# Gadersd/stable-diffusion-burn

Measured on AMD Instinct MI355X. Metric: images/sec @512x512, 20-step DDIM CFG=7.5, SD v1.4, higher is better.
Workload: dtype f32

## Files before the change

### stable_diffusion_burn_amd/csrc/engine.cpp

```cpp
#include "engine.hpp"
#include "mpk_reader.hpp"

#include <dlfcn.h>

#include <algorithm>
#include <cmath>
#include <cstdarg>
#include <cstdio>
#include <cstring>
#include <fstream>
#include <sstream>

namespace sdmi {

static constexpr size_t kAlign = 256;
static constexpr size_t kSlabMin = (size_t)1 << 30;

DevPool::~DevPool() {
    for (auto& s : slabs_) (void)hipFree(s.base);
}

void* DevPool::alloc(size_t bytes) {
    if (bytes == 0) bytes = kAlign;
    bytes = (bytes + kAlign - 1) / kAlign * kAlign;
// ... 782 lines not shown
        for (int i = 0; ok && i < e.ndim; ++i) ok = t.shape[i] == e.dims[i];
        if (!ok) {
            std::ostringstream os;
            os << "load_weights_mpk: '" << t.name << "' has shape [";
            for (size_t i = 0; i < t.shape.size(); ++i) os << (i ? "," : "") << t.shape[i];
            os << "], the configured model expects [";
            for (int i = 0; i < e.ndim; ++i) os << (i ? "," : "") << e.dims[i];
            os << "]";
            throw Error(SDMI_ERR_WEIGHTS, os.str());
        }
        upload_weight(e, reinterpret_cast<const float*>(t.data));
        ++used;
    }
    if (!used) throw Error(SDMI_ERR_WEIGHTS, std::string("load_weights_mpk: no tensor of ") + path + " matches the configured model");
    SDMI_HIP(hipStreamSynchronize(stream_));
    stager_release();
}

void Engine::finalize_weights() {
    int total[3] = {0, 0, 0}, set[3] = {0, 0, 0};
    const WeightEntry* missing[3] = {nullptr, nullptr, nullptr};
    for (auto& e : entries_) {
        ++total[e.group];
        if (e.set) ++set[e.group];
        else if (!missing[e.group]) missing[e.group] = &e;
    }
    if (missing[0]) throw Error(SDMI_ERR_WEIGHTS, "finalize_weights: tensor '" + missing[0]->name + "' was never set");
    static const char* const kGroupName[3] = {"", "CLIP", "VAE encoder"};
    for (int g = 1; g < 3; ++g)
        if (set[g] && missing[g])
            throw Error(SDMI_ERR_WEIGHTS, std::string("finalize_weights: ") + kGroupName[g] + " weights are partially set; missing '" + missing[g]->name + "'");
    SDMI_HIP(hipStreamSynchronize(stream_));
    stager_release();
    clip_ready_ = total[1] > 0 && set[1] == total[1];
    enc_ready_ = total[2] > 0 && set[2] == total[2];
    finalized_ = true;
}

template <class Sink>
static size_t read_npy_f32(const std::string& path, Sink&& sink) {
    std::ifstream f(path, std::ios::binary);
    if (!f) throw Error(SDMI_ERR_IO, "cannot open " + path);
    char magic[8];
    f.read(magic, 8);
    if (!f || std::memcmp(magic, "\x93NUMPY", 6) != 0) throw Error(SDMI_ERR_IO, "not an npy file: " + path);
    uint32_t hlen = 0;
    if (magic[6] == 1) { uint16_t h16; f.read((char*)&h16, 2); hlen = h16; }
    else { f.read((char*)&hlen, 4); }
    std::string header(hlen, ' ');
    f.read(&header[0], hlen);
    if (header.find("'<f4'") == std::string::npos && header.find("\"<f4\"") == std::string::npos)
        throw Error(SDMI_ERR_IO, "npy dtype is not <f4: " + path);
    if (header.find("'fortran_order': True") != std::string::npos) throw Error(SDMI_ERR_IO, "fortran-order npy: " + path);
    const std::streampos start = f.tellg();
    f.seekg(0, std::ios::end);
    const size_t n = (size_t)(f.tellg() - start) / sizeof(float);
    f.seekg(start);
    float* dst = sink(n);
    f.read((char*)dst, (std::streamsize)(n * sizeof(float)));
    if (!f) throw Error(SDMI_ERR_IO, "short read: " + path);
    return n;
}

void Engine::load_weights_dir(const char* dir) {
    if (!dir) throw Error(SDMI_ERR_INVALID, "load_weights_dir: null path");
    SDMI_HIP(hipSetDevice(cfg_.device));
    const bool have_clip = std::ifstream(std::string(dir) + "/clip/token_embedding/weight.npy").good();
    const bool have_enc = std::ifstream(std::string(dir) + "/autoencoder/encoder/conv_in/weight.npy").good();
    for (auto& m : meta_) {
// ... 83 lines not shown
            SDMI_HIP(hipStreamWaitEvent(stream_, ev_user_, 0));
        } else {
            SDMI_HIP(hipDeviceSynchronize());
        }
    }
    SDMI_HIP(hipEventRecord(ev0_, stream_));
}
void Engine::end_call() {
    SDMI_HIP(hipEventRecord(ev1_, stream_));
    if (call_dev_ && has_user_stream_) SDMI_HIP(hipStreamWaitEvent(user_stream_, ev1_, 0));
    SDMI_HIP(hipEventSynchronize(ev1_));
    float ms = 0;
    SDMI_HIP(hipEventElapsedTime(&ms, ev0_, ev1_));
    last_ms = ms; last_kernels = n_kernels_; last_flops = flops_;
}
void Engine::abort_call() noexcept {
    (void)hipStreamSynchronize(stream_);
    try {
        us_ = UNetState{};
        pool_.free_since(call_mark_);
    } catch (...) {}
}

void Engine::set_option(const std::string& key, const std::string& value) {
    if (key == "gemm_tile") opt_force_tile_ = (value == "auto") ? -1 : std::stoi(value);
    else if (key == "splitk") opt_force_splits_ = std::stoi(value);
    else if (key == "roctx") roctx_enable(std::stoi(value) != 0);
    else if (key == "fp8_convs") opt_fp8_convs_ = std::stoi(value);
    else if (key == "fp8_min_rows") opt_fp8_min_rows_ = std::stoi(value);
    else if (key == "fp8_linear") opt_fp8_linear_ = std::stoi(value);
    else if (key == "fp8_ops") opt_fp8_ops_ = std::stoi(value);
    else if (key == "op_resid") opt_op_resid_ = std::stoi(value);
    else if (key == "cfg_share") opt_cfg_share_ = std::stoi(value);
    else if (key == "attn_kv_splits") opt_attn_kv_splits_ = std::stoi(value);
    else if (key == "attn_kv_prefer8") opt_attn_kv_prefer8_ = std::stoi(value);
    else if (key == "b3_grouped") {
        if (!entries_.empty() && std::any_of(entries_.begin(), entries_.end(), [](const WeightEntry& w) { return w.set; }))
            throw Error(SDMI_ERR_STATE, "b3_grouped selects the layout the weight planes are packed in: set it before the first weight is loaded");
        opt_b3_grouped_ = std::stoi(value);
    }
    else if (key == "attn_pack_tail") opt_attn_pack_tail_ = (value == "default") ? 3 : std::stoi(value);
    else if (key == "gn32_min_wgs") opt_gn32_min_wgs_ = (opt_gn32_min_wgs_ & ~0xFFFF) | (std::stoi(value) & 0xFFFF);
    else if (key == "gn32_stats_min_wgs") opt_gn32_min_wgs_ = (opt_gn32_min_wgs_ & 0xFFFF) | ((std::stoi(value) + 1) << 16);
    else if (key == "gn_target_wgs") gn_tune_.target_wgs = std::stoi(value);
    else if (key == "gn_max_threads") gn_tune_.max_threads = std::stoi(value);
    else if (key == "gn_unroll") gn_tune_.unroll = std::stoi(value);
    else if (key == "fp8_tile") opt_fp8_tile_ = (value == "auto") ? -1 : std::stoi(value);
    else if (key == "resid_acc") opt_resid_acc_ = std::stoi(value);
    else if (key == "attn_bf16") opt_attn_bf16_ = std::stoi(value);
    else if (key == "attn_bf16_variant") opt_attn_bf16_variant_ = (value == "default") ? kAttnBf16VariantDefault : std::stoi(value, nullptr, 0);
    else if (key == "attn_split") opt_attn_split_ = std::stoi(value);
    else if (key == "gemm_bf16x") opt_gemm_bf16x_ = std::stoi(value);
    else if (key == "gemm_x32") opt_gemm_x32_ = std::stoi(value);
    else if (key == "gemm_f32s") opt_gemm_f32s_ = std::stoi(value);
    else if (key == "bench_cold") opt_bench_cold_ = std::stoi(value);
    else if (key == "gemm_probe") opt_gemm_probe_ = std::stoi(value);
    else if (key == "conv3_reuse") opt_conv3_reuse_ = std::stoi(value);
    else if (key == "gemm_planes") opt_gemm_planes_ = (value == "default") ? kGemmPlanesDefault : std::stoi(value);
    else if (key == "gemm3x_variant") opt_gemm3x_variant_ = (value == "default") ? kGemm3xVariantDefault : std::stoi(value);
    else if (key == "gemm_bf16x_variant") opt_gemm_bf16x_variant_ = (value == "default") ? kGemmBf16xVariantDefault : std::stoi(value);
    else if (key == "geglu_fuse") opt_geglu_fuse_ = std::stoi(value);
    else if (key == "record_shapes") { record_shapes_ = std::stoi(value) != 0; if (record_shapes_) { shape_counts_.clear(); choice_counts_.clear(); } }
    else if (key == "dump_shapes") {
        std::ofstream f(value);
        if (!f) throw Error(SDMI_ERR_IO, "dump_shapes: cannot write " + value);
        for (auto& kv : shape_counts_) f << kv.first << " " << kv.second << "\n";
// ... 153 lines not shown
    p.Bt3 = in_dt ? nullptr : split_planes(p.Bt);
    p.b3_grouped = b3_grouped((long long)p.N * (p.geglu ? 2 : 1)) ? 1 : 0;
    p.variant = in_dt ? opt_gemm_bf16x_variant_ : opt_gemm3x_variant_;
    const bool s_ok = x32_ok && p.Bt3 && (unsigned long long)p.N * (p.geglu ? 2 : 1) * (unsigned long long)p.kt_total * 192ull < 0xFFFFFF00ull;
    const bool p_ok = s_ok && (unsigned long long)p.NB * p.Hs * p.Ws * (unsigned long long)(p.A3 ? p.a3_ld : p.Cin * 6) < 0xFFFFFF00ull;
    const bool from_planes = !in_dt && p.A3 != nullptr;
    if (from_planes && !p_ok)
        throw Error(s_ok ? SDMI_ERR_UNSUPPORTED : SDMI_ERR_STATE,
                    s_ok ? "fp32 GEMM: an activation tensor stored as bf16 planes (6 bytes per element) reaches 4 GiB (32-bit piece offsets): lower the batch (at 64x64x960 the CFG "
                           "batch 2n must stay <= 182) or set option gemm_planes=0"
                         : "gemm: activation planes given for a layer the plane kernel does not take");
    if (!from_planes && !p.A) throw Error(SDMI_ERR_STATE, "gemm: no activations");
    auto usable = [&](int cfg) { return cfg < 100 || (in_dt ? opt_gemm_bf16x_ != 0 : (cfg >= 300 ? p_ok : cfg >= 200 ? (opt_gemm_f32s_ != 0 && s_ok) : (opt_gemm_x32_ != 0 && x32_ok))); };
    const auto it2 = in_dt ? tuned_mfma_.end() : tuned_mfma_.find(key);
    if (from_planes) {
        const auto itp = tuned_p_.find(key);
        const bool even = p.geglu != 0;
        if (itp != tuned_p_.end() && !(even && (itp->second.cfg == 300 || itp->second.cfg == 303 || itp->second.cfg == 307))) tc = itp->second;
        else tc = choose_tile_p(p.M, p.N, p.kt_total, even);
    }
    else if (it != table.end() && usable(it->second.cfg)) tc = it->second;
    else if (it2 != tuned_mfma_.end() && usable(it2->second.cfg)) tc = it2->second;
    else tc = in_dt ? choose_tile_bf16(p.M, p.N, p.kt_total) : choose_tile(p.M, p.N, p.kt_total, x32_ok, s_ok);
    bool tile_forced = false;
    if (opt_force_tile_ >= 0 && (from_planes ? opt_force_tile_ >= 300 : (opt_force_tile_ < 100 || in_dt || (opt_force_tile_ >= 300 ? p_ok : opt_force_tile_ >= 200 ? s_ok : x32_ok)))) { tc.cfg = opt_force_tile_; tile_forced = true; }
    if (opt_force_splits_ > 0) tc.splits = opt_force_splits_;
    if (force_cfg >= 0) { tc.cfg = force_cfg; tile_forced = true; }
    if (!in_dt && !from_planes && p_ok && opt_gemm_planes_ == 2 && tc.cfg >= 200 && tc.cfg < 200 + kNumGemmTilesS) {
        static const int kSplitToP[kNumGemmTilesS] = {300, 303, 301, 302, 303, 304};
        const int c = kSplitToP[tc.cfg - 200];
        if (!p.geglu || c == 301 || c == 302 || c == 304) tc.cfg = c;
    }
    if (from_planes && tc.cfg < 300) throw Error(SDMI_ERR_STATE, "gemm: activation planes need a plane tile (300 + x)");
    if (force_splits > 0) tc.splits = force_splits;
    if (!in_dt && p.out_mode == 2) tc.splits = 1;
    int splits = std::max(1, std::min(tc.splits, p.kt_total));
    p.kt_per_split = (p.kt_total + splits - 1) / splits;
    splits = (p.kt_total + p.kt_per_split - 1) / p.kt_per_split;
    p.splits = splits;
    const double flops = 2.0 * p.M * (double)p.N * p.K * (p.geglu ? 2.0 : 1.0);
    const unsigned long long es = in_dt ? 2ull : 4ull;
    const unsigned long long a_ext = ((unsigned long long)p.NB * p.Hs * p.Ws - 1) * (unsigned long long)p.a_ld * es + (unsigned long long)p.Cin * es;
    const unsigned long long b_ext = ((unsigned long long)p.N * (p.geglu ? 2 : 1) - 1) * (unsigned long long)p.b_ld * es + (unsigned long long)p.K * es;
    p.zero_page = zero_page_;
    if (in_dt && opt_conv3_reuse_ && !tile_forced && (tc.cfg == 100 || tc.cfg == 101) && conv_gemm_bf16t_supported(p)) tc.cfg += kNumGemmTilesX;
    if (record_shapes_) {
        char ck[128];
        std::snprintf(ck, sizeof ck, "%d,%d,%d k%d s%d u%d W%d cfg=%d splits=%d%s", p.M, p.N, p.K, p.KH, p.stride, p.ups, p.Ws, tc.cfg, splits, p.Bt3 || in_dt ? "" : " (no planes)");
        ++choice_counts_[ck];
    }
    if (tc.cfg >= 300 ? (in_dt || tc.cfg - 300 >= kNumGemmTilesP || !p_ok)
        : tc.cfg >= 200 ? (in_dt || tc.cfg - 200 >= kNumGemmTilesS || !s_ok) : (tc.cfg >= 100 && (tc.cfg - 100 >= (in_dt ? kNumGemmTilesXB : kNumGemmTilesX) || (!in_dt && !x32_ok))))
        throw Error(SDMI_ERR_INVALID, "gemm: large-tile kernel index out of range or not applicable to this layer");
    if (a_ext >= 0xFFFFFFE0ull || b_ext >= 0xFFFFFFE0ull) throw Error(SDMI_ERR_UNSUPPORTED, "GEMM: operand larger than 4 GiB (the buffer-load range check needs 32-bit extents)");
    p.a_bytes = (unsigned)a_ext;
    p.b_bytes = (unsigned)b_ext;
    void* const c3_want = in_dt ? nullptr : p.C3;
    const int ldc3_want = p.ldc3;
    const bool vec_out = (p.N % 4 == 0) && (!p.C || p.ldc % 4 == 0) && (!p.resid || p.ldr % 4 == 0);
    const bool c3_native = c3_want && tc.cfg >= 200 && vec_out && (!p.geglu || (p.geglu == 2 && tc.cfg >= 300));
    std::unique_ptr<Buf> c_tmp;
    if (!c3_native) {
        p.C3 = nullptr;
        if (c3_want && !p.C) {
            c_tmp.reset(new Buf(this, (size_t)p.M * p.N * sizeof(float)));
            p.C = c_tmp->f(); p.ldc = p.N;
// ... 280 lines not shown
            g.out_mode = dt ? 1 : 0;
            launch_gemm(g, dt);
            if (dt) { ProfScope ps_o(this, PC_OTHER); SDMI_HIP(launch_softmax_rows_f32_to_bf16(s.f(), pb.p, nq, nkb, scale * scale, stream_)); }
            else { ProfScope ps_o(this, PC_OTHER); SDMI_HIP(launch_softmax_rows(s.f(), nq, nkb, scale * scale, stream_)); }
            count_kernel();
            if (dt) { ProfScope ps_o(this, PC_OTHER); SDMI_HIP(launch_transpose2d_bf16(vb, vt.p, nkb, d_head, ldv, stream_)); }
            else { ProfScope ps_o(this, PC_OTHER); SDMI_HIP(launch_transpose2d(vb, vt.f(), nkb, d_head, ldv, stream_)); }
            count_kernel();
            ConvGemm g2{};
            g2.A = dt ? pb.f() : s.f(); g2.Bt = vt.f(); g2.C = ob;
            g2.M = nq; g2.N = d_head; g2.K = nkb; g2.NB = 1; g2.Hs = 1; g2.Ws = nq; g2.Cin = nkb; g2.Ho = 1; g2.Wo = nq;
            g2.KH = g2.KW = 1; g2.stride = 1; g2.ldc = ldo; g2.ldr = ldo; g2.a_ld = nkb; g2.b_ld = nkb; g2.CS = 32;
            launch_gemm(g2, dt);
        }
    }
}

void Engine::res_block(const ResW& w, const Act& x, Act& y, int step) {
    Range rng(this, "ResBlock");
    Act h2 = new_act(x.n, x.h, x.w, w.cout);
    const float* rowvec = nullptr;
    if (w.has_embed) rowvec = us_.temb.at(w.temb_index) + (size_t)step * w.cout;
    if (use_fp8(w.conv_in, x)) {
        ActQ q1 = new_actq(x.n, x.h, x.w, x.c);
        group_norm_fp8(w.norm_in, x, q1, true);
        conv_fp8(w.conv_in, q1, h2, rowvec, nullptr);
        release(q1);
    } else {
        Act h1 = plane_gemm(x.c, w.cout) ? new_act3(x.n, x.h, x.w, x.c, 2) : new_act(x.n, x.h, x.w, x.c);
        group_norm(w.norm_in, x, h1, true);
        conv(w.conv_in, h1, h2, 1, 0, rowvec, 0, nullptr);
        release(h1);
    }
    Act sk{};
    if (w.has_skip) {
        if (y.p) { sk = y; sk.p3 = nullptr; sk.view = true; }
        else sk = new_act(y.n, y.h, y.w, y.c);
        if (use_fp8_wide(w.skip.bt8, x.rows()) && x.dt == 1 && x.c % 32 == 0) {
            ActQ xq = new_actq(x.n, x.h, x.w, x.c);
            quantize(x, xq);
            conv_fp8(w.skip, xq, sk, nullptr, nullptr);
            release(xq);
        } else {
            conv(w.skip, x, sk, 1, 0, nullptr, 0, nullptr);
        }
    }
    const Act* resid = w.has_skip ? &sk : &x;
    if (use_fp8(w.conv_out, h2)) {
        ActQ q3 = new_actq(x.n, x.h, x.w, w.cout);
        group_norm_fp8(w.norm_out, h2, q3, true);
        release(h2);
        conv_fp8(w.conv_out, q3, y, nullptr, resid);
        release(q3);
    } else {
        Act h3 = plane_gemm(w.cout, w.cout) ? new_act3(x.n, x.h, x.w, w.cout, 2) : new_act(x.n, x.h, x.w, w.cout);
        group_norm(w.norm_out, h2, h3, true);
        release(h2);
        conv(w.conv_out, h3, y, 1, 0, nullptr, 0, resid);
        release(h3);
    }
    if (w.has_skip) release(sk);
}

bool Engine::use_fp8(const ConvW& w, const Act& x) const {
    return fp8_ && opt_fp8_convs_ && w.bt8 && x.dt == 1 && x.rows() >= opt_fp8_min_rows_;
}

ActQ Engine::new_actq(int n, int h, int w, int c) {
    ActQ a; a.n = n; a.h = h; a.w = w; a.c = c; a.cp = (c + 127) / 128 * 128;
    a.q = pool_.alloc((size_t)a.rows() * a.cp);
    a.s = pool_.alloc((size_t)a.rows() * (a.cp / 32));
    return a;
}
void Engine::release(ActQ& a) {
    if (a.q) pool_.free(a.q);
    if (a.s) pool_.free(a.s);
    a.q = a.s = nullptr;
}

void Engine::group_norm_fp8(const NormW& w, const Act& x, ActQ& y, bool silu) {
    const int hw = x.h * x.w;
    if (x.dt != 1 || y.c != x.c) throw Error(SDMI_ERR_STATE, "group_norm_fp8: bf16 input of matching width expected");
    Buf part(this, gn_partials_bytes_bf16(x.n, hw, x.c, gn_tune_));
    ProfScope ps(this, PC_GROUP_NORM, 0, (double)x.bytes() + (double)x.rows() * (y.cp + y.cp / 32), 2);
    SDMI_HIP(launch_group_norm_fp8(x.p, y.q, y.s, w.gamma, w.beta, x.n, hw, x.c, x.stride(), 32, w.eps, silu, part.p, stream_, &gn_tune_));
    count_kernel(); count_kernel();
}

void Engine::conv_fp8(const ConvW& w, const ActQ& x, Act& y, const float* rowvec, const Act* resid, int stride, int ups) {
    if (x.c != w.cin || (w.k != 3 && w.k != 1) || !w.bt8) throw Error(SDMI_ERR_STATE, "conv_fp8: not an MXFP8-packed convolution");
    const int pad = w.k == 3 ? 1 : 0;
    const int hin = x.h << ups, win = x.w << ups;
    const int ho = (hin + 2 * pad - w.k) / stride + 1, wo = (win + 2 * pad - w.k) / stride + 1;
    if (y.n != x.n || y.h != ho || y.w != wo || y.c != w.cout || y.dt != 1) throw Error(SDMI_ERR_INVALID, "conv_fp8: output shape / type mismatch");
// ... 987 lines not shown
```

### stable_diffusion_burn_amd/csrc/engine.hpp

```cpp
#pragma once
#include <hip/hip_runtime.h>

#include <map>
#include <memory>
#include <stdexcept>
#include <string>
#include <vector>

#include "../../include/sdmi.h"
#include "error.hpp"
#include "kernels.hpp"

namespace sdmi {

#define SDMI_HIP(expr)                                                                                   \
    do {                                                                                                 \
        hipError_t _e = (expr);                                                                          \
        if (_e != hipSuccess)                                                                            \
            throw ::sdmi::Error(SDMI_ERR_HIP, std::string(#expr) + ": " + hipGetErrorString(_e) + " (" + \
                                                  __FILE__ + ":" + std::to_string(__LINE__) + ")");      \
    } while (0)

class DevPool {
public:
// ... 12 lines not shown
    struct Live { int slab; size_t size; unsigned long long serial; };
    std::map<void*, Live> live_;
    size_t reserved_ = 0, in_use_ = 0, high_ = 0;
    unsigned long long serial_ = 0;
};

struct Act {
    float* p = nullptr;
    int n = 0, h = 0, w = 0, c = 0;
    int dt = 0;
    int ld = 0;
    bool view = false;
    void* p3 = nullptr;
    int ld3 = 0;
    size_t bytes3() const { return (size_t)rows() * (size_t)(c / 32) * 192; }
    long long rows() const { return (long long)n * h * w; }
    int stride() const { return ld ? ld : c; }
    size_t bytes() const { return (size_t)rows() * c * (dt ? 2 : 4); }
};

struct ConvW { float* bt = nullptr; float* bias = nullptr; int cin = 0, cout = 0, k = 1; int dt = 0; float* bt8 = nullptr; float* bs8 = nullptr; };
struct ActQ {
    void* q = nullptr; void* s = nullptr;
    int n = 0, h = 0, w = 0, c = 0, cp = 0;
    long long rows() const { return (long long)n * h * w; }
};
struct LinW { float* bt = nullptr; float* bias = nullptr; int cin = 0, cout = 0; int dt = 0; float* bt8 = nullptr; float* bs8 = nullptr; };
struct NormW { float* gamma = nullptr; float* beta = nullptr; int c = 0; float eps = 1e-5f; };

struct ResW {
    NormW norm_in; ConvW conv_in; LinW lin_embed; NormW norm_out; ConvW conv_out; ConvW skip;
    bool has_skip = false, has_embed = false;
    int cin = 0, cout = 0, temb_index = -1;
};
struct MhaW { LinW q, k, v, out; };
struct SpatialW {
    NormW norm; ConvW proj_in, proj_out; NormW ln1, ln2, ln3; MhaW attn1, attn2; LinW geglu_proj, mlp_lin;
    int c = 0, ctx_index = -1;
};
enum BlockKind { BK_CONV, BK_DOWN, BK_RES, BK_RES_ST, BK_RES_UP, BK_RES_ST_UP };
struct UBlock { BlockKind kind; int cin, cout; ConvW conv; ResW res; SpatialW st; ConvW up; };
struct VaeAttnW { NormW norm; ConvW q, k, v, proj_out; int c = 0; };
struct DecBlockW { ResW res[3]; ConvW upsampler; bool has_up = false; int cin = 0, cout = 0; };

struct ClipBlockW { NormW attn_ln, mlp_ln; LinW q, k, v, out, fc1, fc2; };

struct WeightEntry {
    std::string name;
    int kind;
    int ndim;
    int64_t dims[4];
    float** dst;
    int wdt = 0;
    int group = 0;
    float** dst8 = nullptr;
    float** dsts = nullptr;
    float pre_scale = 1.f;
    bool set = false;
};

struct MetaEntry { std::string name; int n; float expect[2]; float* store; };

struct TileChoice { int cfg; int splits; };

class Engine {
public:
// ... 79 lines not shown
    struct SplitRegion { char* base; size_t bytes; char* planes; };
    std::vector<SplitRegion> split_regions_;
    const void* split_planes(const float* bt) const;
    bool b3_grouped(long long rows) const { return opt_b3_grouped_ != 0 && rows % 16 == 0; }
    struct TempSplit {
        Engine* e; const float* bt; void* planes = nullptr;
        TempSplit(Engine* e_, const float* bt_, long long rows, long long K);
        ~TempSplit();
        TempSplit(const TempSplit&) = delete;
        TempSplit& operator=(const TempSplit&) = delete;
    };
    const float* temp_split_bt_ = nullptr;
    const void* temp_split_planes_ = nullptr;
    char* stage_reserve(size_t bytes, size_t* offset, int* half);
    void stage_commit(WeightEntry& e, size_t offset, int half);
    void upload_weight(WeightEntry& e, const float* data);
    void stager_release();
    void ensure_arena(int group);
    bool set_meta(const std::string& name, const float* values, size_t n);
    void add_meta(const std::string& name, int n, float e0, float e1, float* store);
    std::vector<MetaEntry> meta_;
    std::map<std::string, int> meta_index_;
    void add_entry(const std::string& name, int kind, std::initializer_list<int64_t> dims, float** dst, int wdt = 0);
    int cur_group_ = 0;
    void build_model();

    Act new_act(int n, int h, int w, int c, int dt = -1);
    Act new_act3(int n, int h, int w, int c, int what);
    void release(Act& a);
    void probe_report(void* pb_dev, size_t max_blocks, int n, int cin, int h, int w, int cout, int k, int tile_cfg, int splitk);
    void conv(const ConvW& w, const Act& x, Act& y, int stride, int ups, const float* rowvec, int rowvec_stride,
              const Act* resid, bool pad_br = false);
    static Act slice(const Act& parent, int c_off, int c);
    void gemm(const float* A, int a_rows, const float* bt, const float* bias, int cin, int cout, float* C, int ldc,
              const float* resid, int ldr, int dt = -1, int out_mode = 0, const void* A3 = nullptr, void* C3 = nullptr);
    bool plane_gemm(int cin, int cout) const { return !bf16_ && opt_gemm_planes_ != 0 && opt_gemm_f32s_ != 0 && cin % 32 == 0 && cout >= 32; }
    void launch_gemm(ConvGemm& p, int in_dt, int force_cfg = -1, int force_splits = 0);
    int edt() const { return bf16_ ? 1 : 0; }
    size_t esz() const { return bf16_ ? 2 : 4; }
    static float* adv(const float* p, long long elems, int dt) { return (float*)((char*)const_cast<float*>(p) + elems * (dt ? 2 : 4)); }
    TileChoice choose_tile(int M, int N, int kt_total, bool allow_x = false, bool allow_s = false) const;
    void group_norm(const NormW& w, const Act& x, Act& y, bool silu);
    ActQ new_actq(int n, int h, int w, int c);
    void release(ActQ& a);
    void group_norm_fp8(const NormW& w, const Act& x, ActQ& y, bool silu);
    void conv_fp8(const ConvW& w, const ActQ& x, Act& y, const float* rowvec, const Act* resid, int stride = 1, int ups = 0);
    bool use_fp8(const ConvW& w, const Act& x) const;
    bool use_fp8_wide(const float* bt8, long long rows) const { return fp8_ && opt_fp8_convs_ && opt_fp8_linear_ && bt8 && rows >= opt_fp8_min_rows_; }
    void launch_fp8(ConvGemm& p, double flops);
    void gemm_fp8(const ActQ& x, const LinW& w, int n_rows_w, void* C, int ldc, const float* resid, int ldr);
    void conv_raw(const ConvW& w, const Act& x, Act& y, int stride, int ups);
    void quantize(const Act& x, ActQ& y);
    void layer_norm_fp8(const NormW& w, const float* x, long long rows, ActQ& y);
    ActQ new_rowsq(long long rows, int c) { return new_actq(1, 1, (int)rows, c); }
    void layer_norm(const NormW& w, const float* x, long long rows, float* y, int dt = -1, void* y3 = nullptr);
    void gemm_geglu(const float* x, long long rows, const float* bt, const float* bias, int cin, int hidden, float* out, int dt,
                    const void* x3 = nullptr, void* out3 = nullptr);
    void attention(const float* q, int ldq, long long q_bs, const float* k, int ldk, long long k_bs, const float* v,
                   int ldv, long long v_bs, float* o, int ldo, long long o_bs, int n, int nq, int nk, int n_head,
                   int d_head, const int* kv_len_dev, const int* kv_len_host, const float* mask, int mask_ld, int dt = -1, void* o3 = nullptr, bool q_log2 = false);
    static bool q_prescaled(int dt, int d_head) { return dt != 0 && attn_bf16_q_is_log2(d_head); }

    void res_block(const ResW& w, const Act& x, Act& y, int step);
    void spatial_transformer(const SpatialW& w, const Act& x, Act& y);
    void vae_attn(const VaeAttnW& w, const Act& x, Act& y);

// ... 28 lines not shown
    void prof_calibrate();
    double prof_overhead_ms_ = 0;
    void prof_reset() { prof_flush(); for (auto& p : prof_) p = ProfStat{}; prof_tags_.clear(); }
    std::map<std::string, ProfStat> prof_tags_;

private:
    struct ProfScope {
        Engine* e; int cls; double flops, bytes; int n_launch; hipEvent_t a = nullptr, b = nullptr; int tag = -1;
        ProfScope(Engine* e_, int cls_, double flops_ = 0, double bytes_ = 0, int n_launch_ = 1);
        ~ProfScope();
        void set_tag(const char* fmt, ...) __attribute__((format(printf, 2, 3)));
    };
    struct ProfPending { int cls; hipEvent_t a, b; double flops, bytes; int n_launch; int tag; };
    bool prof_tagging_ = false;
    std::vector<std::string> prof_tag_names_;
    std::map<std::string, int> prof_tag_ids_;
    hipEvent_t prof_event();
    bool profiling_ = false;
    std::vector<hipEvent_t> prof_free_;
    std::vector<ProfPending> prof_pending_;

    sdmi_config cfg_;
    bool bf16_ = false;
    bool fp8_ = false;
    int opt_fp8_convs_ = 1;
    int opt_fp8_min_rows_ = 1024;
    int opt_fp8_tile_ = -1;
    int opt_gn32_min_wgs_ = 256 | ((64 + 1) << 16);
    GnTune gn_tune_;
    int opt_b3_grouped_ = 1;
    int opt_attn_pack_tail_ = 3;
    int opt_attn_kv_prefer8_ = 1;
    int opt_attn_kv_splits_ = 0;
    int opt_cfg_share_ = 1;
    int opt_op_resid_ = 0;
    int opt_fp8_ops_ = 0;
    int opt_fp8_linear_ = 0;
    hipStream_t stream_ = nullptr;
    hipEvent_t ev0_ = nullptr, ev1_ = nullptr, ev_user_ = nullptr;
    hipStream_t user_stream_ = nullptr;
    bool has_user_stream_ = false;
    bool call_dev_ = false;
    unsigned long long call_mark_ = 0;
    DevPool pool_;
    std::vector<WeightEntry> entries_;
    std::map<std::string, int> entry_index_;
    std::vector<void*> weight_allocs_;
    bool finalized_ = false;
    std::vector<float> alphas_;

    LinW lin1_time_, lin2_time_;
    std::vector<UBlock> in_blocks_, out_blocks_;
    ResW mid_res1_, mid_res2_;
    SpatialW mid_st_;
    NormW unet_norm_out_;
    ConvW unet_conv_out_;
    std::vector<ResW*> res_list_;
    std::vector<SpatialW*> st_list_;
    ConvW post_quant_, dec_conv_in_, dec_conv_out_;
    ResW dec_mid1_, dec_mid2_;
    VaeAttnW dec_attn_;
    DecBlockW dec_blocks_[4];
    NormW dec_norm_out_;
    float* clip_tok_ = nullptr;
    float* clip_pos_ = nullptr;
    std::vector<ClipBlockW> clip_blocks_;
// ... 63 lines not shown
```

### stable_diffusion_burn_amd/csrc/k_gemm3p.hip

```cpp
#include "kernels.hpp"
#include "k_common.hpp"
#include "k_gemm_epi.hpp"
#include "k_split3.hpp"

namespace sdmi {

typedef float f32x4 __attribute__((ext_vector_type(4)));
typedef unsigned int u32x4 __attribute__((ext_vector_type(4)));
typedef unsigned int u32x2 __attribute__((ext_vector_type(2)));
typedef __bf16 bf16x8 __attribute__((ext_vector_type(8)));
typedef __attribute__((address_space(3))) void lds_void;
typedef __attribute__((address_space(1))) const void global_cvoid;

static const GemmTileInfo kTilesP[kNumGemmTilesP] = {
    {256, 160, "256x160p"}, {256, 128, "256x128p"}, {128, 256, "128x256p"}, {128, 160, "128x160p"}, {128, 128, "128x128p"},
    {64, 64, "64x64p"}, {64, 128, "64x128p"}, {64, 320, "64x320p"}, {128, 64, "128x64p"}};
const GemmTileInfo& gemm_tile_info_p(int cfg) { return kTilesP[cfg]; }

template <int MI, int NI, int NAG, int NBW, int A_BYTES, int NWV>
struct P3Wave {
    static constexpr int NA = 3 * NAG;
    static constexpr int NP = NA + NBW;
    static constexpr int NMF = 6 * NI;
    static constexpr int NAF = MI > 2 ? 3 : MI;
    static_assert(MI == 2 || MI == 4, "fragment rows per wave");
    static_assert(NI >= 2, "plane reads of a fragment take three instruction slots (behind())");

    f32x4 acc[MI][NI];
    u32x4 wf[3][NI];
    u32x4 af[NAF][3];
    int a_iy0[NAG], a_ix0[NAG];
    unsigned a_off[NAG];
    unsigned w_off[NBW];
    unsigned w_kstep;
    const char *Abase, *Wbase, *zero, *a_src;
    unsigned pix_bytes;
    int Hin, Win, ups, Ws, KH, KW, wave;
    int cs, ky, kx, kt_next, kt_end;
    const unsigned char* a_tile;
    const unsigned char* w_tile;
    unsigned char* next_stage;

    template <int J>
    __device__ __forceinline__ void piece() {
        if constexpr (J < NA) {
            constexpr int jg = J / 3, pl = J - 3 * jg;
            if constexpr (pl == 0) {
                const int iy = a_iy0[jg] + ky;
                const int ix = a_ix0[jg] + kx;
                const bool ok = ((unsigned)iy < (unsigned)Hin) & ((unsigned)ix < (unsigned)Win);
                const unsigned off = a_off[jg] + (unsigned)((iy >> ups) * Ws + (ix >> ups)) * pix_bytes + (unsigned)cs * 192u;
                a_src = (ok ? Abase : zero) + (ok ? off : 0u);
            }
            __builtin_amdgcn_global_load_lds((global_cvoid*)(a_src + pl * 64), (lds_void*)(next_stage + ((wave + NWV * jg) * 3 + pl) * 1024), 16, 0, 0);
        } else {
            constexpr int j = J - NA;
            const char* src = Wbase + (w_off[j] + (unsigned)kt_next * w_kstep);
            __builtin_amdgcn_global_load_lds((global_cvoid*)src, (lds_void*)(next_stage + A_BYTES + (wave + NWV * j) * 1024), 16, 0, 0);
        }
        if constexpr (J == NP - 1) {
            const bool adv = kt_next + 1 < kt_end;
            const bool wrap_x = (kx + 1 == KW);
            const bool wrap_y = wrap_x && (ky + 1 == KH);
            const int kx1 = wrap_x ? 0 : kx + 1;
            const int ky1 = wrap_x ? (wrap_y ? 0 : ky + 1) : ky;
            const int cs1 = wrap_y ? cs + 1 : cs;
            kx = adv ? kx1 : kx;
            ky = adv ? ky1 : ky;
            cs = adv ? cs1 : cs;
            kt_next = adv ? kt_next + 1 : kt_next;
        }
    }
    template <int J0, int J1>
    __device__ __forceinline__ void pieces() {
        if constexpr (J0 < J1) { piece<J0>(); pieces<J0 + 1, J1>(); }
    }

    template <int F, int PL>
    __device__ __forceinline__ void read_a() { af[F % NAF][PL] = *reinterpret_cast<const u32x4*>(a_tile + (F * 3 + PL) * 1024); }
    template <int PL, int N>
    __device__ __forceinline__ void read_w() { wf[PL][N] = *reinterpret_cast<const u32x4*>(w_tile + (N * 3 + PL) * 1024); }

    static constexpr int DMA_SLOTS = 3 * NI + NMF;
    template <int MIDX, int K>
    __device__ __forceinline__ void behind() {
        constexpr int pr = K / NI, ni = K % NI;
        if constexpr (MIDX == 0) {
            if constexpr (pr == 0) { read_w<0, ni>(); if constexpr (ni == NI - 1) read_a<0, 2>(); }
            if constexpr (pr == 1) { read_w<1, ni>(); if constexpr (ni == NI - 1) read_a<0, 1>(); }
            if constexpr (K >= 2 * NI && K < 2 * NI + 3) read_a<1, K - 2 * NI>();
            if constexpr (MI > 2 && K >= 2 * NI + 3 && K < 2 * NI + 6) read_a<2, K - 2 * NI - 3>();
        } else if constexpr (MIDX + 2 < MI) {
            if constexpr (K < 3) read_a<MIDX + 2, K>();
        }
        if constexpr (MIDX == 0 && pr >= 3) {
            constexpr int slot = K - 3 * NI;
            pieces<slot * NP / DMA_SLOTS, (slot + 1) * NP / DMA_SLOTS>();
        } else if constexpr (MIDX == 1) {
            constexpr int slot = 3 * NI + K;
            pieces<slot * NP / DMA_SLOTS, (slot + 1) * NP / DMA_SLOTS>();
        }
    }
// ... 44 lines not shown

    const int tid = threadIdx.x;
    const int lane = tid & 63;
    const int wave = __builtin_amdgcn_readfirstlane(tid >> 6);
    const int wm = wave / WN;
    const int wn = wave - wm * WN;

    constexpr int WNC = 16 * NI;
    const bool geglu = p.geglu != 0;
    const int BNO = geglu ? BN / 2 : BN;
    const int MT = (p.M + BM - 1) / BM;
    const int NT = (p.N + BNO - 1) / BNO;
    const GemmWork gw = gemm_work_of_block(p, MT, NT);
    if (!gw.live) return;
    const int lid = gw.lid;
    const int m0 = gw.tm * BM;
    const int n0 = gw.tn * BNO;
    const int z = gw.z;
    const int kt_begin = z * p.kt_per_split;
    const int kt_end = min(kt_begin + p.kt_per_split, p.kt_total);
    const int n_t = kt_end - kt_begin;
    const int T = p.KH * p.KW;
    const int HoWo = p.Ho * p.Wo;

    P3Wave<MI, NI, NAG, NBW, A_BYTES, NWV> w;
    w.Hin = p.Hs << p.ups;
    w.Win = p.Ws << p.ups;
    w.ups = p.ups;
    w.Ws = p.Ws;
    w.KH = p.KH;
    w.KW = p.KW;
    w.wave = wave;
    w.pix_bytes = (unsigned)p.a3_ld;
    w.Abase = reinterpret_cast<const char*>(p.A3);
    w.Wbase = reinterpret_cast<const char*>(p.Bt3);
    w.zero = reinterpret_cast<const char*>(p.zero_page);
    w.a_src = w.zero;

    const int r16 = lane >> 2;
    const int ch = (lane & 3) ^ ((-(r16 >> 2)) & 3);
#pragma unroll
    for (int j = 0; j < NAG; ++j) {
        const int m = m0 + (wave + NWV * j) * 16 + r16;
        const bool ok = m < p.M;
        const int mm = ok ? m : 0;
        const int nb = mm / HoWo;
        const int rem = mm - nb * HoWo;
        const int oy = rem / p.Wo;
        const int ox = rem - oy * p.Wo;
        w.a_off[j] = (unsigned)nb * (unsigned)(p.Hs * p.Ws) * w.pix_bytes + ch * 16;
        w.a_iy0[j] = ok ? oy * p.stride - p.pad : -(1 << 28);
        w.a_ix0[j] = ox * p.stride - p.pad;
    }
    const unsigned w_row_bytes = (unsigned)p.kt_total * 192u;
#pragma unroll
    for (int j = 0; j < NBW; ++j) {
        const int q = wave + NWV * j;
        const int f = q / 3, pl = q - 3 * f;
        int n = n0 + f * 16 + r16;
        long long wrow = n;
        if (p.geglu == 2) {
            const int fw = f / NI, ni = f - fw * NI;
            const int vg = fw / (WN / 2 > 0 ? WN / 2 : 1), col = fw - vg * (WN / 2);
            n = n0 + col * WNC + ni * 16 + r16;
            wrow = (long long)n + (vg ? p.N : 0);
        } else if (geglu) {
            const int fw = f / NI, ni = f - fw * NI;
            n = n0 + fw * (WNC / 2) + (ni >> 1) * 16 + r16;
            wrow = (long long)n + ((ni & 1) ? p.N : 0);
        }
        if (n >= p.N) wrow -= (n - (p.N - 1));
        w.w_off[j] = p.b3_grouped ? (unsigned)(wrow >> 4) * (w_row_bytes * 16u) + pl * 1024 + (unsigned)(wrow & 15) * 64 + ch * 16
                                  : (unsigned)wrow * w_row_bytes + pl * 64 + ch * 16;
    }
    w.w_kstep = p.b3_grouped ? 3072u : 192u;

    w.cs = kt_begin / T;
    const int tap0 = kt_begin - w.cs * T;
    w.ky = tap0 / p.KW;
    w.kx = tap0 - w.ky * p.KW;
    w.kt_next = kt_begin;
    w.kt_end = kt_end;

    const int c15 = lane & 15, g4 = lane >> 4;
    const int fr = c15 * 64 + ((g4 ^ ((-(c15 >> 2)) & 3)) << 4);
    const int a_fr = wm * MI * 3 * 1024 + fr;
    const int w_fr = A_BYTES + wn * NI * 3 * 1024 + fr;

#pragma unroll
    for (int mi = 0; mi < MI; ++mi)
#pragma unroll
        for (int ni = 0; ni < NI; ++ni) w.acc[mi][ni] = f32x4{0.f, 0.f, 0.f, 0.f};

    unsigned long long pt0 = 0, pt1 = 0, pc0 = 0, pwait = 0;
    if constexpr (PROBE) pt0 = __builtin_amdgcn_s_memrealtime();
    w.next_stage = smem_p3;
    w.template pieces<0, NAG * 3 + NBW>();
    if constexpr (PROBE) {
        __syncthreads();
        pt1 = __builtin_amdgcn_s_memrealtime();
        pc0 = __builtin_amdgcn_s_memtime();
    }
    if constexpr (NSTG == 2) {
        for (int t = 0; t < n_t; ++t) {
            const int cur = t & 1;
            unsigned long long pa = 0;
            if constexpr (PROBE) pa = __builtin_amdgcn_s_memtime();
            sdmi_dma_landed();
            __syncthreads();
            if constexpr (PROBE) pwait += __builtin_amdgcn_s_memtime() - pa;
            w.next_stage = smem_p3 + (cur ^ 1) * STAGE;
            w.a_tile = smem_p3 + cur * STAGE + a_fr;
            w.w_tile = smem_p3 + cur * STAGE + w_fr;
// ... 24 lines not shown

    gemm_epilogue_f32<MI, NI, WM, WN>(p, w.acc, smem_p3, m0, n0, z, lid, wave, lane, HoWo);
    if constexpr (PROBE) {
        asm volatile("s_waitcnt vmcnt(0)" ::: "memory");
        __syncthreads();
        unsigned long long* d = p.probe + 24ull * (blockIdx.x + (unsigned long long)gridDim.x * blockIdx.z);
        if (lane == 0) { d[4 + 2 * wave] = pc2 - pc0; d[5 + 2 * wave] = pwait; }
        if (tid == 0) { d[0] = pt0; d[1] = pt1; d[2] = pt2; d[3] = __builtin_amdgcn_s_memrealtime(); }
    }
}

template <int MI, int NI, int WM, int WN, int NSTG, bool PROBE = false>
static hipError_t launch_cfg_3p(const ConvGemm& p, dim3 grid, hipStream_t stream) {
    auto k = conv_gemm3p_kernel<MI, NI, WM, WN, NSTG, PROBE>;
    constexpr int NWV = WM * WN;
    constexpr size_t stage = (size_t)(MI * WM) * 3 * 1024 + (size_t)((NI * WN * 3 + NWV - 1) / NWV) * NWV * 1024;
    constexpr size_t lds = NSTG * stage > (size_t)NWV * 16 * (16 * NI + 4) * 4 ? NSTG * stage : (size_t)NWV * 16 * (16 * NI + 4) * 4;
    static_assert(lds <= 160 * 1024, "the stages must fit the CU's LDS");
    hipError_t e = set_max_dynamic_lds(reinterpret_cast<const void*>(k), (int)lds);
    if (e != hipSuccess) return e;
    hipLaunchKernelGGL(k, grid, dim3(NWV * 64), lds, stream, p);
    return hipGetLastError();
}

hipError_t launch_conv_gemm3p(const ConvGemm& p, int cfg, hipStream_t stream) {
    if (cfg < 0 || cfg >= kNumGemmTilesP) return hipErrorInvalidValue;
    if ((p.Cin % 32) || p.CS != 32 || !p.zero_page || !p.Bt3 || !p.A3 || p.a3_ld <= 0 || (p.a3_ld % 192) || p.out_mode != 0) return hipErrorInvalidValue;
    const bool odd_ni = (cfg == 0 || cfg == 3 || cfg == 7);
    if (p.geglu == 1 && (odd_ni || p.splits != 1 || (p.N & 7) || (p.ldc & 7) || p.rowvec || p.resid)) return hipErrorInvalidValue;
    if (p.geglu == 2 && (cfg == 8 || p.splits != 1 || (p.N & 3) || (p.C && (p.ldc & 3)) || (p.C3 && (p.N & 31)) || p.rowvec || p.resid || (!p.C && !p.C3))) return hipErrorInvalidValue;
    if (p.geglu != 0 && p.geglu != 1 && p.geglu != 2) return hipErrorInvalidValue;
    if ((unsigned long long)p.N * (p.geglu ? 2 : 1) * (unsigned long long)p.kt_total * 192ull >= 0xFFFFFF00ull) return hipErrorInvalidValue;
    if ((unsigned long long)p.NB * p.Hs * p.Ws * (unsigned long long)p.a3_ld >= 0xFFFFFF00ull) return hipErrorInvalidValue;
    const int bm = kTilesP[cfg].bm, bn = kTilesP[cfg].bn;
    const int bno = p.geglu ? bn / 2 : bn;
    const int MT = (p.M + bm - 1) / bm, NT = (p.N + bno - 1) / bno;
    const dim3 grid = gemm_grid(p, MT * NT);
    if (p.probe) {
        if ((unsigned long long)grid.x * grid.z > (unsigned long long)kGemmProbeBlocks) return hipErrorInvalidValue;
        switch (cfg) {
            case 0: return launch_cfg_3p<4, 5, 4, 2, 2, true>(p, grid, stream);
            case 3: return launch_cfg_3p<2, 5, 4, 2, 2, true>(p, grid, stream);
            case 4: return launch_cfg_3p<2, 4, 4, 2, 3, true>(p, grid, stream);
        }
        return hipErrorInvalidValue;
    }
    switch (cfg) {
        case 0: return launch_cfg_3p<4, 5, 4, 2, 2>(p, grid, stream);
        case 1: return launch_cfg_3p<4, 4, 4, 2, 2>(p, grid, stream);
        case 2: return launch_cfg_3p<4, 4, 2, 4, 2>(p, grid, stream);
        case 3: return launch_cfg_3p<2, 5, 4, 2, 2>(p, grid, stream);
        case 4: return launch_cfg_3p<2, 4, 4, 2, 3>(p, grid, stream);
        case 5: return launch_cfg_3p<2, 2, 2, 2, 3>(p, grid, stream);
        case 6: return launch_cfg_3p<2, 4, 2, 2, 2>(p, grid, stream);
        case 7: return launch_cfg_3p<4, 5, 1, 4, 2>(p, grid, stream);
        case 8: return launch_cfg_3p<2, 4, 4, 1, 2>(p, grid, stream);
    }
    return hipErrorInvalidValue;
}

__global__ void split3_rows_kernel(const float* __restrict__ x, unsigned short* __restrict__ y3, long long rows, int kt, long long ld, long long ld3_elems) {
    const long long total = rows * kt * 4;
    for (long long i = (long long)blockIdx.x * blockDim.x + threadIdx.x; i < total; i += (long long)gridDim.x * blockDim.x) {
        const int g = (int)(i & 3);
        const long long rk = i >> 2;
        const long long row = rk / kt;
// ... 50 lines not shown
```

### stable_diffusion_burn_amd/csrc/kernels.hpp

```cpp
#pragma once
#include <hip/hip_runtime.h>
#include <stdint.h>

namespace sdmi {

struct ConvGemm {
    const float* A;
    const float* Bt;
    const void* Bt3;
    int b3_grouped;
    const void* A3;
    int a3_ld;
    float* C;
    void* C3;
    int ldc3;
    float* slabs;
    const float* bias;
    const float* rowvec;
    const float* resid;
    int M, N, K;
    int NB, Hs, Ws, Cin;
    int Ho, Wo;
    int KH, KW, stride, pad, ups;
    int ldc, ldr;
    int a_ld;
    int b_ld;
    int rowvec_stride;
    int CS;
    int kt_total;
    int kt_per_split;
    int splits;
    long long slab_stride;
    unsigned a_bytes, b_bytes;
    int out_mode;
    const void* zero_page;
    const void* a_scale;
    const void* b_scale;
    int variant;
    int resid_acc;
    int geglu;
    unsigned long long* probe;
};

constexpr int kGemmProbeBlocks = 1 << 13;

// ... 136 lines not shown
```

### stable_diffusion_burn_amd/csrc/tuning_table_planes.inc

```
{"262144,128,1152", 304, 1},
{"262144,3,1152", 308, 1},
{"1,1280,1280", 305, 8},
{"1,320,1280", 305, 8},
{"1,640,1280", 305, 8},
{"128,10240,1280", 304, 3},
{"128,1280,1280", 305, 6},
{"128,3840,1280", 304, 8},
{"512,10240,1280", 300, 2},
{"512,1280,1280", 304, 6},
{"512,3840,1280", 301, 4},
{"8192,320,1280", 300, 4},
{"65536,256,2304", 301, 1},
{"262144,256,2304", 301, 1},
{"262144,128,256", 301, 1},
{"262144,128,2304", 301, 1},
{"2048,640,2560", 300, 8},
{"1,1280,320", 305, 1},
{"8192,2560,320", 300, 1},
{"8192,320,320", 308, 1},
{"8192,960,320", 301, 1},
{"4096,512,4096", 301, 4},
{"4096,4096,512", 301, 1},
{"16384,512,4608", 301, 1},
{"65536,512,4608", 301, 1},
// ... 18 lines not shown
{"2048,640,11520", 300, 8},
{"128,1280,1280", 305, 6},
{"128,1280,11520", 303, 32},
{"512,1280,11520", 300, 16},
{"512,1280,1920", 304, 6},
{"512,1280,17280", 300, 16},
{"2048,640,1920", 304, 3},
{"2048,640,17280", 300, 8},
{"512,1280,2560", 304, 6},
{"512,1280,23040", 300, 16},
{"128,1280,2560", 305, 6},
{"128,1280,23040", 303, 32},
{"2048,640,320", 305, 1},
{"2048,640,2880", 304, 3},
{"8192,320,320", 308, 1},
{"8192,320,2880", 300, 4},
{"2048,320,2880", 308, 6},
{"8192,4,2880", 305, 4},
{"512,1280,640", 305, 1},
{"512,1280,5760", 300, 16},
{"2048,640,640", 305, 1},
{"2048,640,5760", 300, 8},
{"8192,640,5760", 300, 2},
{"512,640,5760", 308, 12},
{"8192,320,640", 308, 1},
{"8192,320,5760", 300, 4},
{"2048,640,960", 305, 1},
{"2048,640,8640", 300, 8},
{"8192,320,960", 300, 4},
{"8192,320,8640", 300, 4},
{"4096,320,2880", 300, 8},
{"4096,320,320", 305, 1},
{"4096,960,320", 304, 1},
```

Baseline: 4.049.

## Fold ResNet 1x1 skip conv into the 3x3 output conv as K extension

For ResNet blocks with a 1x1 skip projection, the skip weights are concatenated onto the 3x3 conv_out weights along K and the biases are summed at finalize time. The plane GEMM kernel gains a K-extension path that reads the block input's activation planes for the trailing K tiles. This removes a separate skip GEMM launch, its output buffer write and the residual read. The cost is extra weight memory, more complex address logic in the hot load loop, and new tuning entries for the extended shapes.

Result: no change. 4.076, median of 6 (+0.7%).

```diff
diff --git a/stable_diffusion_burn_amd/csrc/engine.cpp b/stable_diffusion_burn_amd/csrc/engine.cpp
--- a/stable_diffusion_burn_amd/csrc/engine.cpp
+++ b/stable_diffusion_burn_amd/csrc/engine.cpp
@@ -838,9 +838,41 @@
             throw Error(SDMI_ERR_WEIGHTS, std::string("finalize_weights: ") + kGroupName[g] + " weights are partially set; missing '" + missing[g]->name + "'");
     SDMI_HIP(hipStreamSynchronize(stream_));
     stager_release();
+    build_skip_folds();
     clip_ready_ = total[1] > 0 && set[1] == total[1];
     enc_ready_ = total[2] > 0 && set[2] == total[2];
     finalized_ = true;
+}
+
+void Engine::build_skip_folds() {
+    if (bf16_) return;
+    auto fold = [&](ResW& r) {
+        if (!r.has_skip || r.conv_out.k != 3 || r.skip.k != 1 || r.conv_out.dt || r.skip.dt || r.cout % 32 || r.cin % 32) return;
+        const long long rows = r.cout, k_out = 9LL * r.cout, K = k_out + r.cin;
+        if (!r.fold_bt) {
+            void *bt = nullptr, *pl = nullptr, *bias = nullptr;
+            SDMI_HIP(hipMalloc(&bt, (size_t)rows * K * 4));
+            weight_allocs_.push_back(bt);
+            SDMI_HIP(hipMalloc(&pl, (size_t)rows * K * 6));
+            weight_allocs_.push_back(pl);
+            SDMI_HIP(hipMalloc(&bias, (size_t)rows * 4));
+            weight_allocs_.push_back(bias);
+            split_regions_.push_back(SplitRegion{reinterpret_cast<char*>(bt), (size_t)rows * K * 4, reinterpret_cast<char*>(pl)});
+            r.fold_bt = reinterpret_cast<float*>(bt);
+            r.fold_bias = reinterpret_cast<float*>(bias);
+        }
+        SDMI_HIP(hipMemcpy2DAsync(r.fold_bt, K * 4, r.conv_out.bt, k_out * 4, k_out * 4, rows, hipMemcpyDeviceToDevice, stream_));
+        SDMI_HIP(hipMemcpy2DAsync(r.fold_bt + k_out, K * 4, r.skip.bt, r.cin * 4, r.cin * 4, rows, hipMemcpyDeviceToDevice, stream_));
+        SDMI_HIP(launch_pack_split3(r.fold_bt, const_cast<void*>(split_planes(r.fold_bt)), rows, (int)K, stream_, b3_grouped(rows)));
+        std::vector<float> b0(rows), b1(rows);
+        SDMI_HIP(hipMemcpy(b0.data(), r.conv_out.bias, rows * 4, hipMemcpyDeviceToHost));
+        SDMI_HIP(hipMemcpy(b1.data(), r.skip.bias, rows * 4, hipMemcpyDeviceToHost));
+        for (long long i = 0; i < rows; ++i) b0[i] += b1[i];
+        SDMI_HIP(hipMemcpy(r.fold_bias, b0.data(), rows * 4, hipMemcpyHostToDevice));
+    };
+    for (UBlock& b : in_blocks_) fold(b.res);
+    for (UBlock& b : out_blocks_) fold(b.res);
+    SDMI_HIP(hipStreamSynchronize(stream_));
 }
 
 template <class Sink>
@@ -990,6 +1022,7 @@
     else if (key == "fp8_ops") opt_fp8_ops_ = std::stoi(value);
     else if (key == "op_resid") opt_op_resid_ = std::stoi(value);
     else if (key == "cfg_share") opt_cfg_share_ = std::stoi(value);
+    else if (key == "skip_fold") opt_skip_fold_ = std::stoi(value);
     else if (key == "attn_kv_splits") opt_attn_kv_splits_ = std::stoi(value);
     else if (key == "attn_kv_prefer8") opt_attn_kv_prefer8_ = std::stoi(value);
     else if (key == "b3_grouped") {
@@ -1209,6 +1242,7 @@
         if (!p.geglu || c == 301 || c == 302 || c == 304) tc.cfg = c;
     }
     if (from_planes && tc.cfg < 300) throw Error(SDMI_ERR_STATE, "gemm: activation planes need a plane tile (300 + x)");
+    if (p.kt_ext && (!from_planes || (p.K % 32))) throw Error(SDMI_ERR_STATE, "gemm: a K extension needs the plane kernel");
     if (force_splits > 0) tc.splits = force_splits;
     if (!in_dt && p.out_mode == 2) tc.splits = 1;
     int splits = std::max(1, std::min(tc.splits, p.kt_total));
@@ -1555,8 +1589,10 @@
         conv(w.conv_in, h1, h2, 1, 0, rowvec, 0, nullptr);
         release(h1);
     }
+    const bool fold = opt_skip_fold_ && w.has_skip && w.fold_bt && !x.dt && x.p3 && x.c == w.cin && plane_gemm(w.cout, w.cout) && split_planes(w.fold_bt) &&
+                      !use_fp8(w.conv_out, h2);
     Act sk{};
-    if (w.has_skip) {
+    if (w.has_skip && !fold) {
         if (y.p) { sk = y; sk.p3 = nullptr; sk.view = true; }
         else sk = new_act(y.n, y.h, y.w, y.c);
         if (use_fp8_wide(w.skip.bt8, x.rows()) && x.dt == 1 && x.c % 32 == 0) {
@@ -1568,7 +1604,7 @@
             conv(w.skip, x, sk, 1, 0, nullptr, 0, nullptr);
         }
     }
-    const Act* resid = w.has_skip ? &sk : &x;
+    const Act* resid = fold ? nullptr : w.has_skip ? &sk : &x;
     if (use_fp8(w.conv_out, h2)) {
         ActQ q3 = new_actq(x.n, x.h, x.w, w.cout);
         group_norm_fp8(w.norm_out, h2, q3, true);
@@ -1579,10 +1615,27 @@
         Act h3 = plane_gemm(w.cout, w.cout) ? new_act3(x.n, x.h, x.w, w.cout, 2) : new_act(x.n, x.h, x.w, w.cout);
         group_norm(w.norm_out, h2, h3, true);
         release(h2);
-        conv(w.conv_out, h3, y, 1, 0, nullptr, 0, resid);
+        if (fold) conv_skip_folded(w, h3, x, y);
+        else conv(w.conv_out, h3, y, 1, 0, nullptr, 0, resid);
         release(h3);
     }
-    if (w.has_skip) release(sk);
+    if (w.has_skip && !fold) release(sk);
+}
+
+void Engine::conv_skip_folded(const ResW& w, const Act& h3, const Act& x, Act& y) {
+    if (!h3.p3 || !x.p3 || h3.c != w.cout || x.c != w.cin || y.c != w.cout || x.n != y.n || x.h != y.h || x.w != y.w || h3.rows() != y.rows() || (!y.p && !y.p3))
+        throw Error(SDMI_ERR_STATE, "conv_skip_folded: operand shapes / planes");
+    ConvGemm p{};
+    p.Bt = w.fold_bt; p.bias = w.fold_bias; p.C = y.p;
+    p.A3 = h3.p3; p.a3_ld = h3.ld3;
+    p.A3e = x.p3; p.a3e_ld = x.ld3; p.kt_ext = w.cin / 32;
+    p.C3 = y.p3; p.ldc3 = y.ld3;
+    p.M = (int)y.rows(); p.N = w.cout; p.K = 9 * w.cout + w.cin;
+    p.NB = y.n; p.Hs = y.h; p.Ws = y.w; p.Cin = w.cout; p.Ho = y.h; p.Wo = y.w;
+    p.KH = 3; p.KW = 3; p.stride = 1; p.pad = 1; p.ups = 0;
+    p.ldc = y.stride(); p.ldr = y.stride(); p.a_ld = w.cout; p.b_ld = p.K; p.rowvec_stride = 0;
+    p.CS = 32;
+    launch_gemm(p, 0);
 }
 
 bool Engine::use_fp8(const ConvW& w, const Act& x) const {
diff --git a/stable_diffusion_burn_amd/csrc/engine.hpp b/stable_diffusion_burn_amd/csrc/engine.hpp
--- a/stable_diffusion_burn_amd/csrc/engine.hpp
+++ b/stable_diffusion_burn_amd/csrc/engine.hpp
@@ -68,6 +68,7 @@
     NormW norm_in; ConvW conv_in; LinW lin_embed; NormW norm_out; ConvW conv_out; ConvW skip;
     bool has_skip = false, has_embed = false;
     int cin = 0, cout = 0, temb_index = -1;
+    float* fold_bt = nullptr; float* fold_bias = nullptr;
 };
 struct MhaW { LinW q, k, v, out; };
 struct SpatialW {
@@ -213,6 +214,8 @@
     void conv(const ConvW& w, const Act& x, Act& y, int stride, int ups, const float* rowvec, int rowvec_stride,
               const Act* resid, bool pad_br = false);
     static Act slice(const Act& parent, int c_off, int c);
+    void conv_skip_folded(const ResW& w, const Act& h3, const Act& x, Act& y);
+    void build_skip_folds();
     void gemm(const float* A, int a_rows, const float* bt, const float* bias, int cin, int cout, float* C, int ldc,
               const float* resid, int ldr, int dt = -1, int out_mode = 0, const void* A3 = nullptr, void* C3 = nullptr);
     bool plane_gemm(int cin, int cout) const { return !bf16_ && opt_gemm_planes_ != 0 && opt_gemm_f32s_ != 0 && cin % 32 == 0 && cout >= 32; }
@@ -307,6 +310,7 @@
     int opt_attn_pack_tail_ = 3;
     int opt_attn_kv_prefer8_ = 1;
     int opt_attn_kv_splits_ = 0;
+    int opt_skip_fold_ = 1;
     int opt_cfg_share_ = 1;
     int opt_op_resid_ = 0;
     int opt_fp8_ops_ = 0;
diff --git a/stable_diffusion_burn_amd/csrc/k_gemm3p.hip b/stable_diffusion_burn_amd/csrc/k_gemm3p.hip
--- a/stable_diffusion_burn_amd/csrc/k_gemm3p.hip
+++ b/stable_diffusion_burn_amd/csrc/k_gemm3p.hip
@@ -31,12 +31,15 @@
     u32x4 af[NAF][3];
     int a_iy0[NAG], a_ix0[NAG];
     unsigned a_off[NAG];
+    unsigned e_doff[NAG];
     unsigned w_off[NBW];
     unsigned w_kstep;
     const char *Abase, *Wbase, *zero, *a_src;
-    unsigned pix_bytes;
+    long long e_dbase;
+    unsigned pix_bytes, e_dpix;
     int Hin, Win, ups, Ws, KH, KW, wave;
     int cs, ky, kx, kt_next, kt_end;
+    int kt_e, tap_e;
     const unsigned char* a_tile;
     const unsigned char* w_tile;
     unsigned char* next_stage;
@@ -49,8 +52,9 @@
                 const int iy = a_iy0[jg] + ky;
                 const int ix = a_ix0[jg] + kx;
                 const bool ok = ((unsigned)iy < (unsigned)Hin) & ((unsigned)ix < (unsigned)Win);
-                const unsigned off = a_off[jg] + (unsigned)((iy >> ups) * Ws + (ix >> ups)) * pix_bytes + (unsigned)cs * 192u;
-                a_src = (ok ? Abase : zero) + (ok ? off : 0u);
+                const bool ext = kt_next >= kt_e;
+                const unsigned off = a_off[jg] + (ext ? e_doff[jg] : 0u) + (unsigned)((iy >> ups) * Ws + (ix >> ups)) * (pix_bytes + (ext ? e_dpix : 0u)) + (unsigned)cs * 192u;
+                a_src = ok ? Abase + (ext ? e_dbase : 0ll) + off : zero;
             }
             __builtin_amdgcn_global_load_lds((global_cvoid*)(a_src + pl * 64), (lds_void*)(next_stage + ((wave + NWV * jg) * 3 + pl) * 1024), 16, 0, 0);
         } else {
@@ -65,9 +69,10 @@
             const int kx1 = wrap_x ? 0 : kx + 1;
             const int ky1 = wrap_x ? (wrap_y ? 0 : ky + 1) : ky;
             const int cs1 = wrap_y ? cs + 1 : cs;
-            kx = adv ? kx1 : kx;
-            ky = adv ? ky1 : ky;
-            cs = adv ? cs1 : cs;
+            const bool ext1 = kt_next + 1 >= kt_e;
+            kx = adv ? (ext1 ? tap_e : kx1) : kx;
+            ky = adv ? (ext1 ? tap_e : ky1) : ky;
+            cs = adv ? (ext1 ? kt_next + 1 - kt_e : cs1) : cs;
             kt_next = adv ? kt_next + 1 : kt_next;
         }
     }
@@ -178,7 +183,9 @@
     w.KW = p.KW;
     w.wave = wave;
     w.pix_bytes = (unsigned)p.a3_ld;
+    w.e_dpix = (unsigned)p.a3e_ld - w.pix_bytes;
     w.Abase = reinterpret_cast<const char*>(p.A3);
+    w.e_dbase = p.A3e ? (long long)reinterpret_cast<uintptr_t>(p.A3e) - (long long)reinterpret_cast<uintptr_t>(p.A3) : 0ll;
     w.Wbase = reinterpret_cast<const char*>(p.Bt3);
     w.zero = reinterpret_cast<const char*>(p.zero_page);
     w.a_src = w.zero;
@@ -195,6 +202,7 @@
         const int oy = rem / p.Wo;
         const int ox = rem - oy * p.Wo;
         w.a_off[j] = (unsigned)nb * (unsigned)(p.Hs * p.Ws) * w.pix_bytes + ch * 16;
+        w.e_doff[j] = (unsigned)nb * (unsigned)(p.Hs * p.Ws) * w.e_dpix;
         w.a_iy0[j] = ok ? oy * p.stride - p.pad : -(1 << 28);
         w.a_ix0[j] = ox * p.stride - p.pad;
     }
@@ -221,10 +229,16 @@
     }
     w.w_kstep = p.b3_grouped ? 3072u : 192u;
 
+    w.kt_e = p.kt_total - p.kt_ext;
+    w.tap_e = p.pad;
     w.cs = kt_begin / T;
     const int tap0 = kt_begin - w.cs * T;
     w.ky = tap0 / p.KW;
     w.kx = tap0 - w.ky * p.KW;
+    if (kt_begin >= w.kt_e) {
+        w.cs = kt_begin - w.kt_e;
+        w.ky = w.kx = w.tap_e;
+    }
     w.kt_next = kt_begin;
     w.kt_end = kt_end;
 
@@ -315,6 +329,11 @@
     if (p.geglu != 0 && p.geglu != 1 && p.geglu != 2) return hipErrorInvalidValue;
     if ((unsigned long long)p.N * (p.geglu ? 2 : 1) * (unsigned long long)p.kt_total * 192ull >= 0xFFFFFF00ull) return hipErrorInvalidValue;
     if ((unsigned long long)p.NB * p.Hs * p.Ws * (unsigned long long)p.a3_ld >= 0xFFFFFF00ull) return hipErrorInvalidValue;
+    if (p.kt_ext < 0 || p.kt_ext >= p.kt_total) return hipErrorInvalidValue;
+    if (p.kt_ext && (!p.A3e || p.a3e_ld <= 0 || (p.a3e_ld % 192) || p.a3e_ld < p.kt_ext * 192 || p.geglu || p.ups || p.stride != 1 ||
+                     p.KH != p.KW || p.KH != 2 * p.pad + 1 || p.Ho != p.Hs || p.Wo != p.Ws || (p.kt_total - p.kt_ext) * 32 != p.Cin * p.KH * p.KW))
+        return hipErrorInvalidValue;
+    if (p.kt_ext && (unsigned long long)p.NB * p.Hs * p.Ws * (unsigned long long)p.a3e_ld >= 0xFFFFFF00ull) return hipErrorInvalidValue;
     const int bm = kTilesP[cfg].bm, bn = kTilesP[cfg].bn;
     const int bno = p.geglu ? bn / 2 : bn;
     const int MT = (p.M + bm - 1) / bm, NT = (p.N + bno - 1) / bno;
diff --git a/stable_diffusion_burn_amd/csrc/kernels.hpp b/stable_diffusion_burn_amd/csrc/kernels.hpp
--- a/stable_diffusion_burn_amd/csrc/kernels.hpp
+++ b/stable_diffusion_burn_amd/csrc/kernels.hpp
@@ -11,6 +11,9 @@
     int b3_grouped;
     const void* A3;
     int a3_ld;
+    const void* A3e;
+    int a3e_ld;
+    int kt_ext;
     float* C;
     void* C3;
     int ldc3;
diff --git a/stable_diffusion_burn_amd/csrc/tuning_table_planes.inc b/stable_diffusion_burn_amd/csrc/tuning_table_planes.inc
--- a/stable_diffusion_burn_amd/csrc/tuning_table_planes.inc
+++ b/stable_diffusion_burn_amd/csrc/tuning_table_planes.inc
@@ -74,3 +74,13 @@
 {"4096,320,2880", 300, 8},
 {"4096,320,320", 305, 1},
 {"4096,960,320", 304, 1},
+{"8192,320,3520", 300, 4},
+{"8192,320,3840", 300, 4},
+{"2048,640,6080", 300, 8},
+{"2048,640,6720", 300, 8},
+{"2048,640,7040", 300, 8},
+{"2048,640,7680", 300, 8},
+{"512,1280,12160", 300, 16},
+{"512,1280,13440", 300, 16},
+{"512,1280,14080", 300, 16},
+{"128,1280,14080", 303, 32},
```
